# silvadirceu/acoss-1

Hardware: AMD Instinct MI355X
Metric: song-pairs/sec (CSM+Qmax) on 12-d HPCP, ~2000 frames/track; MAP parity (higher is better)
Workload: dtype f32; 1 GPU; covers80-shaped synthetic HPCP (hard corpus), Serra09 CRP+Qmax, all unordered pairs; tracks=164, frames_per_track=2000, m=9, tau=1, oti=True, parallelism=pair-matrix row stripes dp1

## Files before the change

acoss-1_amd/csrc/crp_split.hip:

```cpp
#include <cstdlib>
#include <cstring>
#include <type_traits>

#include "crp_internal.hpp"

__device__ int acoss_writelane(int value, int lane, int old) __asm("llvm.amdgcn.writelane.i32");

namespace acoss {

namespace {

constexpr int kMS = 9;

constexpr unsigned kNone = 0x7fffu;


struct PairView {
  const float* X;
  const float* X2;
  const float* Yr;
  int nq, nr, tau;
  const float* NXq;
  const float* NXr;
  int Mp, Np;
};

__device__ __forceinline__ PairView pair_view(const CrpBatch& B, int p) {
  PairView v;
  const int ta = B.pairs[2 * p], tb = B.pairs[2 * p + 1];
  v.X = B.feats + B.off[ta] * 12;
  v.X2 = B.feats2 ? B.feats2 + (size_t)ta * B.ldn * 24 : nullptr;
  v.Yr = B.yrot + (size_t)p * B.yrot_stride;
  v.nq = B.len[ta];
  v.nr = B.len[tb];
  v.tau = B.tau;
  v.NXq = B.NX + (size_t)ta * B.ldn;
  v.NXr = B.NX + (size_t)tb * B.ldn;
  const int2 dm = B.dims[p];
  v.Mp = dm.x;
  v.Np = dm.y;
  return v;
}

constexpr int kSR = 32;
struct KeyPlanes {
  uint16_t* hr;
  uint16_t* hc;
};

__device__ __forceinline__ float gram12(const f32x4& x0, const f32x4& x1, const f32x4& x2, const f32x4& y0,
                                        const f32x4& y1, const f32x4& y2) {
  float g = 0.0f;
  g = __builtin_fmaf(x0.x, y0.x, g);
  g = __builtin_fmaf(x0.y, y0.y, g);
  g = __builtin_fmaf(x0.z, y0.z, g);
  g = __builtin_fmaf(x0.w, y0.w, g);
  g = __builtin_fmaf(x1.x, y1.x, g);
  g = __builtin_fmaf(x1.y, y1.y, g);
  g = __builtin_fmaf(x1.z, y1.z, g);
  g = __builtin_fmaf(x1.w, y1.w, g);
  g = __builtin_fmaf(x2.x, y2.x, g);
  g = __builtin_fmaf(x2.y, y2.y, g);
  g = __builtin_fmaf(x2.z, y2.z, g);
  g = __builtin_fmaf(x2.w, y2.w, g);
  return g;
}

__device__ __forceinline__ float cell_gram(const PairView& V, int fq, int fr) {
  const f32x4* x = reinterpret_cast<const f32x4*>(V.X + (size_t)fq * 12);
  const f32x4* y = reinterpret_cast<const f32x4*>(V.Yr + (size_t)fr * 12);
  const f32x4 x0 = x[0], x1 = x[1], x2 = x[2], y0 = y[0], y1 = y[1], y2 = y[2];
  return gram12(x0, x1, x2, y0, y1, y2);
}

__device__ __forceinline__ unsigned cell_finish(const PairView& V, int i, int j, float dot) {
  const float d2 = (V.NXq[i] - 2.0f * dot) + V.NXr[j];
  return __builtin_bit_cast(unsigned, d2 > 0.0f ? d2 : 0.0f);
}

__device__ __forceinline__ unsigned cell_key(const PairView& V, int i, int j) {
  float dot = cell_gram(V, i * V.tau, j * V.tau);
#pragma unroll 1
  for (int u = 1; u < kMS; ++u) dot = dot + cell_gram(V, (i + u) * V.tau, (j + u) * V.tau);
  return cell_finish(V, i, j, dot);
}

template <bool ROW>
struct LineCells {
  static constexpr bool kRow = ROW;
  PairView V;
  int fix;
  __device__ __forceinline__ int qi(int e) const { return ROW ? fix : e; }
  __device__ __forceinline__ int rj(int e) const { return ROW ? e : fix; }
  __device__ __forceinline__ unsigned operator()(int e) const { return cell_key(V, qi(e), rj(e)); }
};

typedef float f32x2 __attribute__((ext_vector_type(2)));
typedef __attribute__((address_space(1))) uint16_t gu16;
__device__ __forceinline__ void st_u16(gu16* base, unsigned idx, unsigned v) {
  typedef __attribute__((address_space(1))) char gchar;
  *(gu16*)((gchar*)base + idx * 2u) = (uint16_t)v;
}

__device__ __forceinline__ f32x2 pk_fma(f32x2 a, f32x2 b, f32x2 c) { return __builtin_elementwise_fma(a, b, c); }

constexpr int kSysCols = 56;
constexpr int kThreads = 256;

__device__ __forceinline__ float dpp_shr1(float v) {
  return __builtin_bit_cast(float, __builtin_amdgcn_mov_dpp(__builtin_bit_cast(int, v), 0x138, 0xf, 0xf, true));
}

template <bool PARTIAL>
__device__ __forceinline__ void sweep_body_sys(const PairView& V, int p, int strip, const KeyPlanes& K, int ldr,
                                               int ldc, int64_t kstride, uint16_t* Hr) {
  constexpr int kSteps = kSR + kMS - 1;
  const int i0 = strip * kSR;
  const int rows = PARTIAL ? min(kSR, V.Mp - i0) : kSR;
  const int lane = threadIdx.x & 63;
  const int w = __builtin_amdgcn_readfirstlane(threadIdx.x >> 6);
  uint16_t* Hc = K.hc + (size_t)p * kstride;
  const float* X2b = V.X2 + (size_t)i0 * 24;
  const float* Nq0 = V.NXq + i0;
  auto nqr = [&](int r) {
    const float* base = Nq0;
    asm volatile("" : "+s"(base));
    return *(const __attribute__((address_space(4))) float*)(base + r);
  };
  auto xpair = [&](int kk, f32x2 (&x)[12]) {
    const float* base = X2b;
    asm volatile("" : "+s"(base));
    const cfloat4* q = (const cfloat4*)(base + kk * 24);
#pragma unroll
    for (int c = 0; c < 6; ++c) {
      const f32x4 v = q[c];
      x[2 * c] = f32x2{v.x, v.y};
      x[2 * c + 1] = f32x2{v.z, v.w};
    }
  };
  auto load_y = [&](int jb, f32x4 (&y)[3]) {
    const int f = min(jb + lane, V.nr - 1);
    const f32x4* src = reinterpret_cast<const f32x4*>(V.Yr + (size_t)f * 12);
    y[0] = src[0];
    y[1] = src[1];
    y[2] = src[2];
  };
  const int nblk = (V.Np + kSysCols - 1) / kSysCols;
  f32x4 ynext[3];
  if (w < nblk) load_y(w * kSysCols, ynext);
#pragma unroll 1
  for (int cb = w; cb < nblk; cb += 4) {
    const int jb = cb * kSysCols;
    float y[12];
#pragma unroll
    for (int q = 0; q < 3; ++q) {
      y[4 * q] = ynext[q].x;
      y[4 * q + 1] = ynext[q].y;
      y[4 * q + 2] = ynext[q].z;
      y[4 * q + 3] = ynext[q].w;
    }
    if (cb + 4 < nblk) load_y(jb + 4 * kSysCols, ynext);
    const int col = jb + lane - (kMS - 1);
    const bool valid = lane >= kMS - 1 && col < V.Np;
    const unsigned hcol = valid ? (unsigned)col : (unsigned)(ldr - 1);
    const float ny = valid ? V.NXr[col] : 0.0f;
    gu16* hrow = (gu16*)Hr;
    float A[kMS];
    unsigned kh[16];
    unsigned hw[16];
    f32x2 xb[12];
    xpair(0, xb);
#pragma unroll
    for (int kk = 0; kk < kSteps; kk += 2) {
      f32x2 g2 = pk_fma(xb[0], f32x2{y[0], y[0]}, f32x2{0.0f, 0.0f});
#pragma unroll
      for (int b = 1; b < 12; ++b) g2 = pk_fma(xb[b], f32x2{y[b], y[b]}, g2);
      if (kk + 2 < kSteps) xpair(kk + 2, xb);
      float dots[2];
#pragma unroll
      for (int h = 0; h < 2; ++h) {
        const int k = kk + h;
        const float g = h ? g2.y : g2.x;
#pragma unroll
        for (int u = kMS - 1; u >= 1; --u) {
          const int r = k - u;
          if (r >= 0 && r < kSR) A[u] = dpp_shr1(A[u - 1]) + g;
        }
        if (k < kSR) A[0] = g;
        dots[h] = A[kMS - 1];
      }
      const int r = kk - (kMS - 1);
      if (r >= 0) {
        const f32x2 nq = f32x2{nqr(r), nqr(r + 1)};
        const f32x2 d2 = pk_fma(f32x2{-2.0f, -2.0f}, f32x2{dots[0], dots[1]}, nq) + f32x2{ny, ny};
        unsigned k0 = __builtin_bit_cast(unsigned, d2.x > 0.0f ? d2.x : 0.0f);
        unsigned k1 = __builtin_bit_cast(unsigned, d2.y > 0.0f ? d2.y : 0.0f);
        if (!PARTIAL || r + 1 < rows) {
          st_u16(hrow, hcol, k0 >> 16);
          st_u16(hrow, (unsigned)ldr + hcol, k1 >> 16);
        } else {
          if (r < rows) st_u16(hrow, hcol, k0 >> 16);
          if (r >= rows) k0 = kNone << 16;
          k1 = kNone << 16;
        }
        hrow += 2 * ldr;
        asm volatile("" : "+s"(hrow));
        if (r < 16) {
          kh[r] = k0;
          kh[r + 1] = k1;
        } else {
          hw[r - 16] = __builtin_amdgcn_perm(k0, kh[r - 16], 0x07060302u);
          hw[r - 15] = __builtin_amdgcn_perm(k1, kh[r - 15], 0x07060302u);
        }
      }
    }
    {
      const int m = lane & 3, b = lane & ~3;
      const bool o1 = (m & 1) != 0, o2 = (m & 2) != 0;
      uint32_t T[4][4];
#pragma unroll
      for (int d = 0; d < 4; ++d) {
        const uint32_t x0 = hw[d], x1 = hw[4 + d], x2 = hw[8 + d], x3 = hw[12 + d];
        uint32_t p0 = dpp_u32<0xB1>(x0, x0), p1 = dpp_u32<0xB1>(x1, x1), p2 = dpp_u32<0xB1>(x2, x2),
                 p3 = dpp_u32<0xB1>(x3, x3);
        asm volatile("" : "+v"(p0), "+v"(p1), "+v"(p2), "+v"(p3));
        const uint32_t y0 = o1 ? p1 : x0, y1 = o1 ? x1 : p0, y2 = o1 ? p3 : x2, y3 = o1 ? x3 : p2;
        uint32_t q0 = dpp_u32<0x4E>(y0, y0), q1 = dpp_u32<0x4E>(y1, y1), q2 = dpp_u32<0x4E>(y2, y2),
                 q3 = dpp_u32<0x4E>(y3, y3);
        asm volatile("" : "+v"(q0), "+v"(q1), "+v"(q2), "+v"(q3));
        T[0][d] = o2 ? q2 : y0;
        T[1][d] = o2 ? q3 : y1;
        T[2][d] = o2 ? y2 : q0;
        T[3][d] = o2 ? y3 : q1;
      }
#pragma unroll
      for (int k = 0; k < 4; ++k) {
        const int c = jb + b + k - (kMS - 1);
        if (b + k >= kMS - 1 && c < V.Np)
          reinterpret_cast<uint4*>(Hc + ((size_t)strip * ldc + c) * kSR)[m] = make_uint4(T[k][0], T[k][1], T[k][2], T[k][3]);
      }
    }
  }
  __syncthreads();
  const int padw = (int)((V.Np + 31) & ~31) - V.Np;
  for (int e = threadIdx.x; e < kSR * 32; e += kThreads) {
    const int r = e >> 5, c = e & 31;
    if (c < padw && r < rows) Hr[(size_t)r * ldr + V.Np + c] = (uint16_t)kNone;
  }
}


__device__ __forceinline__ unsigned pk_min_u16(unsigned a, unsigned b) {
  typedef unsigned short u16x2 __attribute__((ext_vector_type(2)));
  return __builtin_bit_cast(unsigned, __builtin_elementwise_min(__builtin_bit_cast(u16x2, a), __builtin_bit_cast(u16x2, b)));
}
__device__ __forceinline__ unsigned pk_max_u16(unsigned a, unsigned b) {
  typedef unsigned short u16x2 __attribute__((ext_vector_type(2)));
  return __builtin_bit_cast(unsigned, __builtin_elementwise_max(__builtin_bit_cast(u16x2, a), __builtin_bit_cast(u16x2, b)));
}
__device__ __forceinline__ unsigned pk_add_u16(unsigned a, unsigned b) {
  typedef unsigned short u16x2 __attribute__((ext_vector_type(2)));
  return __builtin_bit_cast(unsigned, __builtin_bit_cast(u16x2, a) + __builtin_bit_cast(u16x2, b));
}

__device__ __forceinline__ uint32_t gather_flags(uint32_t acc, uint32_t s, int h) {
  return ((s >> (15 - h)) & (0x00010001u << h)) | acc;
}

__device__ __forceinline__ unsigned pk_subsat_u16(unsigned a, unsigned b) {
  typedef unsigned short u16x2 __attribute__((ext_vector_type(2)));
  return __builtin_bit_cast(unsigned, __builtin_elementwise_sub_sat(__builtin_bit_cast(u16x2, a), __builtin_bit_cast(u16x2, b)));
}

template <int NW>
__device__ __forceinline__ unsigned swar_min_greater(const unsigned (&pv)[NW], unsigned x) {
  const unsigned X = ((0x10000u - x - 1u) & 0xffffu) * 0x10001u;
  unsigned a = 0xffffffffu;
#pragma unroll
  for (int h = 0; h < NW; ++h) a = pk_min_u16(a, pk_add_u16(pv[h], X));
  const unsigned d = min(a & 0xffffu, a >> 16);
  return d < kNone - x - 1u ? d + x + 1u : 0xffffffffu;
}

__device__ __forceinline__ uint32_t gather_flags8(uint32_t acc, uint32_t s, int h) {
  return ((s >> (7 - h)) & (0x01010101u << h)) | acc;
}

typedef __attribute__((address_space(3))) unsigned lds_u32;
struct HistAddr {
  unsigned hb, sk;
  __device__ __forceinline__ explicit HistAddr(unsigned* hist) {
    hb = (unsigned)__builtin_amdgcn_readfirstlane((int)(unsigned)(size_t)(lds_u32*)hist);
    sk = hb + 512u + 4u * (threadIdx.x & 63);
  }
};
__device__ __forceinline__ void hist_add(unsigned* hist, const HistAddr& A, unsigned c, bool in) {
  if (in) __hip_atomic_fetch_add(hist + c, 1u, __ATOMIC_RELAXED, __HIP_MEMORY_SCOPE_WAVEFRONT);
}

template <int NW>
__device__ __forceinline__ bool hist_rank_w8(const unsigned (&w8)[NW], unsigned base8, int rho, unsigned* hist,
                                             unsigned* P, int* le, int* less) {
  const int lane = threadIdx.x & 63;
  reinterpret_cast<uint2*>(hist)[lane] = make_uint2(0u, 0u);
  __builtin_amdgcn_wave_barrier();
  const unsigned cmin = base8 == 0u ? 0u : 1u;
  const HistAddr A(hist);
  const unsigned lane1 = (unsigned)(lane + 1) * 0x01010101u;
  const unsigned hbm = A.hb - 4u;
#pragma unroll
  for (int h = 0; h < NW; ++h) {
    const unsigned wp = w8[h] + 0x01010101u;
    const unsigned H = wp & 0x80808080u;
    const unsigned S = wp + ((H - (H >> 7)) & lane1);
#pragma unroll
    for (int k = 0; k < 4; ++k) {
      const unsigned a = hbm + 4u * ((S >> (8 * k)) & 0xffu);
      __hip_atomic_fetch_add((lds_u32*)(size_t)a, 1u, __ATOMIC_RELAXED, __HIP_MEMORY_SCOPE_WAVEFRONT);
    }
  }
  __builtin_amdgcn_wave_barrier();
  const uint2 hv = reinterpret_cast<const uint2*>(hist)[lane];
  const int sl = (int)(hv.x + hv.y);
  const int S = wave_incl_scan(sl);
  const int tot = __builtin_amdgcn_readlane(S, 63);
  const int r = rho;
  if (r < 0 || r >= tot) return false;
  const int E = S - sl;
  const int src = __builtin_ctzll(__ballot(E <= r && r < S));
  const int Es = __builtin_amdgcn_readlane(E, src);
  const int h0 = __builtin_amdgcn_readlane((int)hv.x, src), h1 = __builtin_amdgcn_readlane((int)hv.y, src);
  const bool second = r >= Es + h0;
  if (cmin && src == 0 && !second) return false;
  *P = base8 + 2u * (unsigned)src + (second ? 1u : 0u);
  *less = Es + (second ? h0 : 0);
  *le = *less + (second ? h1 : h0);
  return true;
}

template <int KPL>
struct Line {
  static_assert(KPL == 32, "split word order assumes 32 elements per lane");
  unsigned pv[KPL / 2];
  unsigned w8[KPL / 4];
  unsigned base8;
  bool win;
  __device__ __forceinline__ void build_window(unsigned center) {
    base8 = center > 63u ? center - 63u : 0u;
    win = true;
    const unsigned B2 = base8 * 0x10001u;
    unsigned c[KPL / 2];
#pragma unroll
    for (int h = 0; h < KPL / 2; ++h) c[h] = pk_min_u16(pk_subsat_u16(pv[h], B2), 0x007f007fu);
#pragma unroll
    for (int h = 0; h < KPL / 4; ++h) w8[h] = __builtin_amdgcn_perm(c[h + 8], c[h], 0x06020400u);
  }
  __device__ __forceinline__ bool in_win(unsigned x) const { return win && x >= base8 && x <= base8 + 126u; }
  __device__ __forceinline__ int ebase() const {
    int e = (threadIdx.x & 63) * KPL;
    asm volatile("" : "+v"(e));
    return e;
  }
  __device__ __forceinline__ int elem(int eb, int b) const { return eb + b; }
  static __device__ __forceinline__ int lane_of(int e) { return e / KPL; }
  static __device__ __forceinline__ int bit_of(int e) { return e % KPL; }
  __device__ __forceinline__ unsigned sample() const { return pv[0] & 0xffffu; }
  __device__ __forceinline__ unsigned pfx(int q) const { return q < 16 ? (pv[q] & 0xffffu) : (pv[q - 16] >> 16); }
  template <bool STORED_SPLIT>
  __device__ __forceinline__ void load_lanes(const uint16_t* col0, size_t lane_stride, int n) {
    const int lane = threadIdx.x & 63;
    const int base = lane * KPL;
    const uint16_t* src = col0 + (base < n ? (size_t)lane * lane_stride : (size_t)0);
    win = false;
    base8 = 0u;
    unsigned w[KPL / 2];
#pragma unroll
    for (int q = 0; q < KPL / 8; ++q) {
      const uint4 v = reinterpret_cast<const uint4*>(src)[q];
      w[4 * q + 0] = v.x;
      w[4 * q + 1] = v.y;
      w[4 * q + 2] = v.z;
      w[4 * q + 3] = v.w;
    }
    if (STORED_SPLIT) {
#pragma unroll
      for (int h = 0; h < KPL / 2; ++h) pv[h] = w[h];
    } else {
#pragma unroll
      for (int h = 0; h < KPL / 2; ++h)
        pv[h] = __builtin_amdgcn_perm(w[8 + (h >> 1)], w[h >> 1], (h & 1) ? 0x07060302u : 0x05040100u);
    }
    if (base >= n) {
#pragma unroll
      for (int h = 0; h < KPL / 2; ++h) pv[h] = kNone * 0x10001u;
    }
  }
  __device__ __forceinline__ unsigned cnt8(unsigned x) const {
    const unsigned X4 = (x - base8 + 0x80u) * 0x01010101u;
    unsigned c = 0;
#pragma unroll
    for (int h = 0; h < KPL / 4; ++h) c = __builtin_popcount((X4 - w8[h]) & 0x80808080u) + c;
    return c;
  }
  __device__ __forceinline__ unsigned cnt16(unsigned x) const {
    const unsigned X2 = (x + 0x8000u) * 0x10001u;
    unsigned c = 0;
#pragma unroll
    for (int h = 0; h < KPL / 2; ++h) c = __builtin_popcount((X2 - pv[h]) & 0x80008000u) + c;
    return c;
  }
  __device__ __forceinline__ int count_le(unsigned x) const {
    if (in_win(x)) {
      const unsigned X4 = (x - base8 + 0x80u) * 0x01010101u;
      unsigned c = 0;
#pragma unroll
      for (int h = 0; h < KPL / 4; ++h) c = __builtin_popcount((X4 - w8[h]) & 0x80808080u) + c;
      return wave_sum((int)c);
    }
    const unsigned X2 = (x + 0x8000u) * 0x10001u;
    unsigned c = 0;
#pragma unroll
    for (int h = 0; h < KPL / 2; ++h) c = __builtin_popcount((X2 - pv[h]) & 0x80008000u) + c;
    return wave_sum((int)c);
  }
  __device__ __forceinline__ bool eq_in_win(unsigned P) const {
    return in_win(P) && (P > base8 || base8 == 0u);
  }
  __device__ __forceinline__ uint32_t eq8(unsigned P) const {
    const unsigned PP = (P - base8) * 0x01010101u;
    uint32_t ne8 = 0;
#pragma unroll
    for (int h = 0; h < KPL / 4; ++h) ne8 = gather_flags8(ne8, (w8[h] ^ PP) + 0x7f7f7f7fu, h);
    return ~ne8;
  }
  __device__ __forceinline__ uint32_t eq16(unsigned P) const {
    const unsigned PP = P * 0x10001u;
    uint32_t ne = 0;
#pragma unroll
    for (int h = 0; h < KPL / 2; ++h) ne = gather_flags(ne, (pv[h] ^ PP) + 0x7fff7fffu, h);
    return ~ne;
  }
  __device__ __forceinline__ uint32_t eq_mask(unsigned P) const {
    if (in_win(P) && (P > base8 || base8 == 0u)) {
      const unsigned PP = (P - base8) * 0x01010101u;
      uint32_t ne8 = 0;
#pragma unroll
      for (int h = 0; h < KPL / 4; ++h) ne8 = gather_flags8(ne8, (w8[h] ^ PP) + 0x7f7f7f7fu, h);
      return ~ne8;
    }
    const unsigned PP = P * 0x10001u;
    uint32_t ne = 0;
#pragma unroll
    for (int h = 0; h < KPL / 2; ++h) ne = gather_flags(ne, (pv[h] ^ PP) + 0x7fff7fffu, h);
    return ~ne;
  }
  __device__ __forceinline__ uint32_t le8(unsigned x) const {
    const unsigned X4 = (x - base8 + 0x80u) * 0x01010101u;
    uint32_t le8 = 0;
#pragma unroll
    for (int h = 0; h < KPL / 4; ++h) le8 = gather_flags8(le8, X4 - w8[h], h);
    return le8;
  }
  __device__ __forceinline__ uint32_t le16(unsigned x) const {
    const unsigned X2 = (x + 0x8000u) * 0x10001u;
    uint32_t le = 0;
#pragma unroll
    for (int h = 0; h < KPL / 2; ++h) le = gather_flags(le, X2 - pv[h], h);
    return le;
  }
  __device__ __forceinline__ uint32_t le_mask(unsigned x) const {
    if (in_win(x)) {
      const unsigned X4 = (x - base8 + 0x80u) * 0x01010101u;
      uint32_t le8 = 0;
#pragma unroll
      for (int h = 0; h < KPL / 4; ++h) le8 = gather_flags8(le8, X4 - w8[h], h);
      return le8;
    }
    const unsigned X2 = (x + 0x8000u) * 0x10001u;
    uint32_t le = 0;
#pragma unroll
    for (int h = 0; h < KPL / 2; ++h) le = gather_flags(le, X2 - pv[h], h);
    return le;
  }
  __device__ __forceinline__ void min_max_lane(unsigned* a_io, unsigned* b_io) const {
    unsigned a = *a_io, b = *b_io;
#pragma unroll
    for (int h = 0; h < KPL / 2; ++h) {
      a = pk_min_u16(a, pv[h]);
      b = pk_max_u16(b, pk_add_u16(pv[h], 0x00010001u) & 0x7fff7fffu);
    }
    *a_io = a;
    *b_io = b;
  }
  __device__ __forceinline__ void min_max(unsigned* mn, unsigned* mx) const {
    unsigned a = 0xffffffffu, b = 0u;
    min_max_lane(&a, &b);
    a = min(a & 0xffffu, a >> 16);
    b = max(b & 0xffffu, b >> 16);
    *mn = wave_min_u32(a);
    const unsigned m = wave_max_u32(b);
    *mx = m ? m - 1 : 0u;
  }
  __device__ __forceinline__ unsigned min_greater_lane(unsigned x) const { return swar_min_greater(pv, x); }
  __device__ __forceinline__ unsigned min_greater(unsigned x) const { return wave_min_u32(min_greater_lane(x)); }
  static constexpr int kHalves = 1;
  static constexpr bool kHist = true;
  __device__ __forceinline__ bool hist_rank(unsigned hint, int rho, unsigned* hist, unsigned* P, int* le,
                                            int* less, unsigned* hbase) const {
    if (win) {
      *hbase = base8;
      return hist_rank_w8(w8, base8, rho, hist, P, le, less);
    }
    const int lane = threadIdx.x & 63;
    const unsigned base = hint > 64u ? hint - 64u : 0u;
    *hbase = base;
    reinterpret_cast<uint2*>(hist)[lane] = make_uint2(0u, 0u);
    __builtin_amdgcn_wave_barrier();
    const HistAddr HA(hist);
    unsigned below = 0;
    if (base > 0u) {
      const unsigned X2 = (base - 1u + 0x8000u) * 0x10001u;
#pragma unroll
      for (int h = 0; h < KPL / 2; ++h) below = __builtin_popcount((X2 - pv[h]) & 0x80008000u) + below;
    }
#pragma unroll
    for (int h = 0; h < KPL / 2; ++h) {
#pragma unroll
      for (int half = 0; half < 2; ++half) {
        const unsigned c = (half ? (pv[h] >> 16) : (pv[h] & 0xffffu)) - base;
        hist_add(hist, HA, c, c < 128u);
      }
    }
    const int below_tot = wave_sum((int)below);
    __builtin_amdgcn_wave_barrier();
    const uint2 hv = reinterpret_cast<const uint2*>(hist)[lane];
    const int sl = (int)(hv.x + hv.y);
    const int S = wave_incl_scan(sl);
    const int tot = __builtin_amdgcn_readlane(S, 63);
    const int r = rho - below_tot;
    if (r < 0 || r >= tot) return false;
    const int E = S - sl;
    const int src = __builtin_ctzll(__ballot(E <= r && r < S));
    const int Es = __builtin_amdgcn_readlane(E, src);
// ... 379 lines not shown
    const float d2 = (nq_me - 2.0f * dot) + nr_me;
    G.key = __builtin_bit_cast(unsigned, d2 > 0.0f ? d2 : 0.0f);
  }
  __builtin_amdgcn_wave_barrier();
  return G;
}

template <class LT, class KF>
__device__ __forceinline__ void group_keys2(const LT& L, unsigned P1, int g1, unsigned P2, int g2, const KF& keyf,
                                            WaveLds& W, Group* G1, Group* G2) {
  const int lane = threadIdx.x & 63;
  const int ebase = L.ebase();
  auto m1 = L.eq_mask(P1);
  auto m2 = L.eq_mask(P2);
  const int c1 = popc(m1), c2 = popc(m2);
  const int packed = c1 | (c2 << 16);
  const int sc = wave_incl_scan(packed) - packed;
  int i1 = sc & 0xffff, i2 = g1 + (sc >> 16);
  while (m1) {
    W.list[i1++] = L.elem(ebase, ctz(m1));
    m1 &= m1 - 1;
  }
  while (m2) {
    W.list[i2++] = L.elem(ebase, ctz(m2));
    m2 &= m2 - 1;
  }
  __builtin_amdgcn_wave_barrier();
  const int g = g1 + g2;
  const int e_me = W.list[lane < g ? lane : 0];
  const float nq_me = keyf.V.NXq[keyf.qi(e_me)], nr_me = keyf.V.NXr[keyf.rj(e_me)];
  for (int t = lane; t < kMS * g; t += 64) {
    const int k = t / kMS, u = t - k * kMS;
    const int e = W.list[k];
    W.gv[t] = cell_gram(keyf.V, (keyf.qi(e) + u) * keyf.V.tau, (keyf.rj(e) + u) * keyf.V.tau);
  }
  __builtin_amdgcn_wave_barrier();
  unsigned key = 0xffffffffu;
  if (lane < g) {
    float dot = W.gv[lane * kMS];
#pragma unroll
    for (int u = 1; u < kMS; ++u) dot = dot + W.gv[lane * kMS + u];
    const float d2 = (nq_me - 2.0f * dot) + nr_me;
    key = __builtin_bit_cast(unsigned, d2 > 0.0f ? d2 : 0.0f);
  }
  __builtin_amdgcn_wave_barrier();
  const int elem = lane < g ? e_me : 0;
  *G1 = Group{P1, g1, elem, lane < g1 ? key : 0xffffffffu, 0};
  *G2 = Group{P2, g2, elem, (lane >= g1 && lane < g) ? key : 0xffffffffu, g1};
}

__device__ __forceinline__ unsigned group_min(const Group& G) {
  return wave_min_u32(G.mine(threadIdx.x & 63) ? G.key : 0xffffffffu);
}

__device__ __forceinline__ unsigned group_rank(const Group& G, int rho) {
  const int lane = threadIdx.x & 63;
  int cl = 0, ce = 0;
  for (int k = 0; k < G.g; ++k) {
    const unsigned o = (unsigned)lane_bcast((int)G.key, k);
    cl += o < G.key;
    ce += o == G.key;
  }
  const bool act = lane < G.g;
  const int src = __builtin_ctzll(__ballot(act && cl <= rho && rho < cl + ce));
  return (unsigned)lane_bcast((int)G.key, src);
}

__device__ __forceinline__ void group_rank2(const Group& G, int rho, unsigned* v0, unsigned* v1) {
  const int lane = threadIdx.x & 63;
  int cl = 0, ce = 0;
  for (int k = 0; k < G.g; ++k) {
    const unsigned o = (unsigned)lane_bcast((int)G.key, k);
    cl += o < G.key;
    ce += o == G.key;
  }
  const bool act = lane < G.g;
  const int s0 = __builtin_ctzll(__ballot(act && cl <= rho && rho < cl + ce));
  const int s1 = __builtin_ctzll(__ballot(act && cl <= rho + 1 && rho + 1 < cl + ce));
  *v0 = (unsigned)lane_bcast((int)G.key, s0);
  *v1 = (unsigned)lane_bcast((int)G.key, s1);
}

template <class LT, class F>
__device__ __forceinline__ void group_rounds(const LT& L, unsigned P, int g, WaveLds& W, F fn) {
  const int lane = threadIdx.x & 63;
  auto m = L.eq_mask(P);
  const int cnt = popc(m);
  int idx = wave_incl_scan(cnt) - cnt;
  const int ebase = L.ebase();
  for (int r0 = 0; r0 < g; r0 += 64) {
    while (m && idx < r0 + 64) {
      const int q = ctz(m);
      m &= m - 1;
      W.list[idx - r0] = L.elem(ebase, q);
      ++idx;
    }
    __builtin_amdgcn_wave_barrier();
    if (lane < min(64, g - r0)) fn(W.list[lane]);
    __builtin_amdgcn_wave_barrier();
  }
}

__device__ __forceinline__ unsigned hist_bin_of_rank(const unsigned* hist, int* rho) {
  const int lane = threadIdx.x & 63;
  const unsigned c0 = hist[4 * lane], c1 = hist[4 * lane + 1], c2 = hist[4 * lane + 2], c3 = hist[4 * lane + 3];
  const int tot = (int)(c0 + c1 + c2 + c3);
  const int ex = wave_incl_scan(tot) - tot;
  const int r = *rho;
  int bin = -1, below = ex;
  if (r >= ex && r < ex + tot) {
    if (r < below + (int)c0) {
      bin = 0;
    } else if (r < below + (int)(c0 + c1)) {
      bin = 1;
      below += c0;
    } else if (r < below + (int)(c0 + c1 + c2)) {
      bin = 2;
      below += c0 + c1;
    } else {
      bin = 3;
      below += c0 + c1 + c2;
    }
  }
  const int src = __builtin_ctzll(__ballot(bin >= 0));
  *rho = r - lane_bcast(below, src);
  return (unsigned)(4 * src + lane_bcast(bin, src));
}

template <class LT, class KF>
__device__ __forceinline__ unsigned big_group_rank(const LT& L, unsigned P, int rho, int g, const KF& keyf, WaveLds& W) {
  const int lane = threadIdx.x & 63;
  unsigned* hist = reinterpret_cast<unsigned*>(W.gv);
  unsigned hi8 = 0, lo8 = 0;
#pragma unroll 1
  for (int pass = 0; pass < 2; ++pass) {
    for (int b = lane; b < 256; b += 64) hist[b] = 0u;
    __builtin_amdgcn_wave_barrier();
    group_rounds(L, P, g, W, [&](int e) {
      const unsigned k = keyf(e);
      if (pass == 0)
        atomicAdd(&hist[(k >> 8) & 0xffu], 1u);
      else if (((k >> 8) & 0xffu) == hi8)
        atomicAdd(&hist[k & 0xffu], 1u);
    });
    __builtin_amdgcn_wave_barrier();
    const unsigned bin = hist_bin_of_rank(hist, &rho);
    __builtin_amdgcn_wave_barrier();
    if (pass == 0)
      hi8 = bin;
    else
      lo8 = bin;
  }
  return (P << 16) | (hi8 << 8) | lo8;
}

template <class LT, class KF>
__device__ __forceinline__ unsigned rank_in_prefix(const LT& L, unsigned P, int rho, int g, const KF& keyf, WaveLds& W,
                                   Group* cache) {
  if (g <= 64) {
    if (cache->g < 0 || cache->P != P) *cache = group_keys(L, P, g, keyf, W);
    return group_rank(*cache, rho);
  }
  return big_group_rank(L, P, rho, g, keyf, W);
}

struct Plan {
  unsigned Pl, hbase, Ph2;
  int le, less, gh2, lo, hi;
  float q, lo_f, hi_f;
  bool found, next_ok, both;
};

template <class LT, class KF>
__device__ __forceinline__ Plan line_plan(const LT& L, int n, float kappa, WaveLds& W, Hint* hint) {
  Plan pl;
  pl.q = (float)(n - 1) * kappa;
  pl.lo_f = floorf(pl.q);
  pl.hi_f = ceilf(pl.q);
  pl.lo = (int)pl.lo_f;
  pl.hi = (int)pl.hi_f;
  const int lo = pl.lo, hi = pl.hi;
  unsigned kmin = 0, kmax = 0x7f80u;
  const bool hinted = hint->P != kNoHint;
  if (!hinted) L.min_max(&kmin, &kmax);
  int le = 0, less = 0;
  int passes = 0;
  unsigned Pl = 0u, hbase = 0u;
  bool found = false;
  if constexpr (LT::kHist) {
    if (hinted) found = L.hist_rank(hint->P, lo, W.hist, &Pl, &le, &less, &hbase);
  }
  if (!found) Pl = prefix_of_rank(L, lo, kmin, kmax, n, hint->P, &le, &less, &passes);
  hint->P = Pl;
  hint->dens = hinted ? 0.5f * hint->dens + 0.5f * (float)(le - less) : (float)(le - less);
  pl.Pl = Pl;
  pl.hbase = hbase;
  pl.le = le;
  pl.less = less;
  pl.found = found;
  pl.Ph2 = 0u;
  pl.gh2 = 0;
  pl.next_ok = hi != lo && hi >= le && found && hist_next(W.hist, hbase, Pl, &pl.Ph2, &pl.gh2);
  pl.both = pl.next_ok && le - less <= 64 && (le - less) + pl.gh2 <= 64;
  return pl;
}

template <class LT, class KF>
__device__ __forceinline__ void line_groups(const LT& L, const Plan& pl, const KF& keyf, WaveLds& W, Group* c_lo,
                                            Group* c_hi, unsigned* vlo_o, unsigned* vhi_o) {
  const unsigned Pl = pl.Pl;
  const int le = pl.le, less = pl.less, lo = pl.lo, hi = pl.hi;
  unsigned vlo, vhi;
  if (pl.both) {
    group_keys2(L, Pl, le - less, pl.Ph2, pl.gh2, keyf, W, c_lo, c_hi);
    vlo = group_rank(*c_lo, lo - less);
    vhi = group_min(*c_hi);
  } else if (hi != lo && hi < le && le - less <= 64) {
    *c_lo = group_keys(L, Pl, le - less, keyf, W);
    group_rank2(*c_lo, lo - less, &vlo, &vhi);
  } else {
    vlo = rank_in_prefix(L, Pl, lo - less, le - less, keyf, W, c_lo);
    vhi = vlo;
  }
  if (!pl.both && hi != lo && !(hi < le && le - less <= 64)) {
    if (hi < le) {
      vhi = rank_in_prefix(L, Pl, hi - less, le - less, keyf, W, c_lo);
    } else {
      unsigned Ph;
      int gh;
      if (pl.next_ok) {
        Ph = pl.Ph2;
        gh = pl.gh2;
      } else {
        Ph = L.min_greater(Pl);
        gh = L.count_le(Ph) - le;
      }
      vhi = rank_in_prefix(L, Ph, 0, gh, keyf, W, c_hi);
    }
  }
  *vlo_o = vlo;
  *vhi_o = vhi;
}

__device__ __forceinline__ void plan_threshold(const Plan& pl, unsigned vlo, unsigned vhi, float* thr, float* T) {
  const float slo = sqrt_rn(__builtin_bit_cast(float, vlo));
  float th;
  if (pl.lo_f == pl.hi_f) {
    th = slo;
  } else {
    const float shi = sqrt_rn(__builtin_bit_cast(float, vhi));
    const float aa = slo * (pl.hi_f - pl.q);
    const float bb = shi * (pl.q - pl.lo_f);
    th = aa + bb;
  }
  *thr = th;
  *T = sq_threshold(th);
}

template <class LT, class KF>
__device__ __forceinline__ void line_threshold(const LT& L, int n, float kappa, const KF& keyf, WaveLds& W, Group* c_lo,
                               Group* c_hi, float* thr, float* T, Hint* hint) {
  const Plan pl = line_plan<LT, KF>(L, n, kappa, W, hint);
  unsigned vlo, vhi;
  line_groups(L, pl, keyf, W, c_lo, c_hi, &vlo, &vhi);
  plan_threshold(pl, vlo, vhi, thr, T);
}

template <class LT, class KF>
__device__ __forceinline__ auto le_bits(const LT& L, unsigned Tbits, const KF& keyf, WaveLds& W, const Group& c_lo,
                            const Group& c_hi) {
  const unsigned T16 = Tbits >> 16;
  const int lane = threadIdx.x & 63;
  const auto word = L.le_mask(T16);
  const bool lo_hit = c_lo.g >= 0 && c_lo.P == T16, hi_hit = c_hi.g >= 0 && c_hi.P == T16;
  W.words[lane] = 0xffffffffu;
  if (LT::kHalves == 2) W.words[64 + lane] = 0xffffffffu;
  __builtin_amdgcn_wave_barrier();
  if (lo_hit || hi_hit) {
    const bool cmine = lo_hit ? c_lo.mine(lane) : c_hi.mine(lane);
    const unsigned ckey = lo_hit ? c_lo.key : c_hi.key;
    const int celem = lo_hit ? c_lo.elem : c_hi.elem;
    if (cmine && ckey > Tbits) atomicAnd(&W.words[LT::lane_of(celem)], ~(1u << LT::bit_of(celem)));
  } else {
    const int g = wave_sum(popc(L.eq_mask(T16)));
    if (g == 0) return word;
    if (g <= 64) {
      const Group G = group_keys(L, T16, g, keyf, W);
      if (lane < G.g && G.key > Tbits) atomicAnd(&W.words[LT::lane_of(G.elem)], ~(1u << LT::bit_of(G.elem)));
    } else {
      group_rounds(L, T16, g, W, [&](int e) {
        if (keyf(e) > Tbits) atomicAnd(&W.words[LT::lane_of(e)], ~(1u << LT::bit_of(e)));
      });
    }
  }
  __builtin_amdgcn_wave_barrier();
  if constexpr (LT::kHalves == 2)
    return word & (((uint64_t)W.words[64 + lane] << 32) | W.words[lane]);
  else
    return word & W.words[lane];
}

constexpr int kRowsLds = 4 * (int)sizeof(WaveLds) + kSR * 64 * 4;
constexpr int kRowsLds2 = 4 * (int)sizeof(WaveLds) + kSR * 128 * 4;

template <int J>
__device__ __forceinline__ void transpose_stage(uint32_t (&a)[32]) {
  constexpr uint32_t m = J == 16 ? 0x0000ffffu : J == 8 ? 0x00ff00ffu : J == 4 ? 0x0f0f0f0fu : J == 2 ? 0x33333333u
                                                                                                      : 0x55555555u;
#pragma unroll
  for (int k = 0; k < 32; ++k) {
    if (k & J) continue;
    const uint32_t t = ((a[k] >> J) ^ a[k + J]) & m;
    a[k + J] ^= t;
    a[k] ^= t << J;
  }
}

__device__ __forceinline__ void transpose32(uint32_t (&a)[32]) {
  transpose_stage<16>(a);
  transpose_stage<8>(a);
  transpose_stage<4>(a);
  transpose_stage<2>(a);
  transpose_stage<1>(a);
}

template <int KQ>
struct LineOf {
  using T = LineS<KQ>;
};
template <>
struct LineOf<0> {
  using T = Line<32>;
};
template <>
struct LineOf<2> {
  using T = Line2;
};

template <int NW, int KQ, int RB>
__device__ __forceinline__ void rows_body(const PairView& V, int p, int strip, const uint16_t* Hr, int ldr,
                                          float kappa, float* __restrict__ thr,
                                          float* __restrict__ Tq, int64_t thr_stride, uint32_t* __restrict__ RT,
                                          int64_t rt_stride, int ld, WaveLds* wl, uint32_t (*rowbits)[RB]) {
  using LT = typename LineOf<KQ>::T;
  const int i0 = strip * kSR;
  const int w = __builtin_amdgcn_readfirstlane(threadIdx.x >> 6), lane = threadIdx.x & 63;
  WaveLds& W = wl[w];
  constexpr int RPW = kSR / NW;
  Hint hint{kNoHint, 1.0f};
  auto load_row = [&](LT& Ld, int i) {
    int64_t rowoff = (int64_t)(i - i0) * ldr;
    asm volatile("" : "+s"(rowoff));
    if constexpr (KQ == 0) {
      Ld.template load_lanes<false>(Hr + rowoff, 32, V.Np);
    } else if constexpr (KQ == 2) {
      Ld.A.template load_lanes<false>(Hr + rowoff, 32, V.Np);
      Ld.B.template load_lanes<false>(Hr + rowoff + 2048, 32, V.Np - 2048);
    } else {
      const uint16_t* row = Hr + rowoff;
      Ld.load([&](int e) { return row + (unsigned)e; }, V.Np);
    }
  };
  constexpr bool kPF = KQ != 2;
  auto row = [&](LT& L, int r, auto&& prefetch) {
    const int i = i0 + r;
    uint64_t word = 0;
    if (i < V.Mp) {
      if (hint.P == kNoHint) hint.P = sample_hint(L, V.Np, kappa, W.hist);
      if constexpr (KQ != 8) {
        if (hint.P != kNoHint) L.build_window(hint.P);
      }
      prefetch();
      const LineCells<true> keyf{V, i};
      float th, T;
      Group c_lo, c_hi;
      c_lo.g = c_hi.g = -1;
      line_threshold(L, V.Np, kappa, keyf, W, &c_lo, &c_hi, &th, &T, &hint);
      if (lane == 0) {
        thr[(size_t)p * thr_stride + i] = th;
        Tq[(size_t)p * thr_stride + i] = T;
      }
      word = le_bits(L, __builtin_bit_cast(unsigned, T), keyf, W, c_lo, c_hi);
      if constexpr (KQ == 8 || KQ == 16) word = lane_words<KQ>((uint32_t)word);
    }
    rowbits[r][lane] = (uint32_t)word;
    if constexpr (KQ == 2) rowbits[r][64 + lane] = (uint32_t)(word >> 32);
  };
  const int r1 = (w + 1) * RPW;
  {
    LT Lnext;
    if (kPF && i0 + w * RPW < V.Mp) load_row(Lnext, i0 + w * RPW);
#pragma unroll 1
    for (int r = w * RPW; r < r1; ++r) {
      LT L;
      if (i0 + r < V.Mp) {
        if constexpr (kPF)
          L = Lnext;
        else
          load_row(L, i0 + r);
      }
      row(L, r, [&] {
        if (kPF && r + 1 < r1 && i0 + r + 1 < V.Mp) load_row(Lnext, i0 + r + 1);
      });
    }
  }
  __syncthreads();
  uint32_t* out = RT + (size_t)p * rt_stride + (size_t)strip * ld;
  for (int b = threadIdx.x; 32 * b < V.Np; b += NW * 64) {
    uint32_t a[32];
#pragma unroll
    for (int r = 0; r < 32; ++r) a[r] = rowbits[r][b];
    transpose32(a);
    uint32_t* o = out + 32 * b;
    if (32 * b + 32 <= ld) {
#pragma unroll
      for (int q = 0; q < 32; q += 4) *reinterpret_cast<uint4*>(o + q) = make_uint4(a[q], a[q + 1], a[q + 2], a[q + 3]);
    } else {
#pragma unroll
      for (int q = 0; q < 32; ++q)
        if (32 * b + q < V.Np) o[q] = a[q];
    }
  }
}


constexpr int kSweepWPE = 4;
struct SweepArgs {
  CrpBatch B;
  KeyPlanes K;
  int ldr, ldc;
  int64_t kstride;
  float kappa;
  float* thr;
  float* Tq;
  int64_t thr_stride;
  uint32_t* RT;
  int64_t rt_stride;
  int ld, short_n;
};
struct ColsArgs {
  CrpBatch B;
  KeyPlanes K;
  int ldc;
  int64_t kstride;
  float kappa;
  const uint32_t* RT;
  float* thr;
  float* Tq;
  int64_t thr_stride;
  uint32_t* maskT;
  int64_t mask_stride;
  int ld, short_n;
};
template <int KQ>
constexpr int kSweepLds = KQ == 2 ? kRowsLds2 : kRowsLds;

template <int KQ>
__device__ __forceinline__ void sweep_rows_block(const SweepArgs& A, int strip, int p, char* smem) {
  constexpr int RB = KQ == 2 ? 128 : 64;
  const CrpBatch& B = A.B;
  const KeyPlanes& K = A.K;
  const int ldr = A.ldr, ldc = A.ldc, ld = A.ld, short_n = A.short_n;
  const int64_t kstride = A.kstride, thr_stride = A.thr_stride, rt_stride = A.rt_stride;
  const float kappa = A.kappa;
  float* thr = A.thr;
  float* Tq = A.Tq;
  uint32_t* RT = A.RT;
  const PairView V = pair_view(B, p);
  const int i0 = strip * kSR;
  if (i0 >= V.Mp || V.Np <= 0) return;
  uint16_t* Hr = K.hr + (size_t)p * kstride + (size_t)i0 * ldr;
  if (i0 + kSR <= V.Mp)
    sweep_body_sys<false>(V, p, strip, K, ldr, ldc, kstride, Hr);
  else
    sweep_body_sys<true>(V, p, strip, K, ldr, ldc, kstride, Hr);
  __syncthreads();
  WaveLds* wl = reinterpret_cast<WaveLds*>(smem);
  uint32_t(*rowbits)[RB] = reinterpret_cast<uint32_t(*)[RB]>(smem + 4 * sizeof(WaveLds));
  if (KQ == 8 || V.Np <= short_n)
    rows_body<4, 8, RB>(V, p, strip, Hr, ldr, kappa, thr, Tq, thr_stride, RT, rt_stride, ld, wl, rowbits);
  else if (KQ == 16)
    rows_body<4, 16, RB>(V, p, strip, Hr, ldr, kappa, thr, Tq, thr_stride, RT, rt_stride, ld, wl, rowbits);
  else if (KQ == 2 && V.Np > 2048)
    rows_body<4, 2, RB>(V, p, strip, Hr, ldr, kappa, thr, Tq, thr_stride, RT, rt_stride, ld, wl, rowbits);
  else
    rows_body<4, 0, RB>(V, p, strip, Hr, ldr, kappa, thr, Tq, thr_stride, RT, rt_stride, ld, wl, rowbits);
}

template <int KQ>
__global__ __launch_bounds__(kThreads, kSweepWPE) void k_sweep_rows9(SweepArgs A) {
  __shared__ __attribute__((aligned(16))) char smem[kSweepLds<KQ>];
  sweep_rows_block<KQ>(A, blockIdx.x, blockIdx.y, smem);
}

constexpr int kCPWLong = 2;
constexpr int kCPWShort = 4;
template <int KQ>
constexpr int kCPW = (KQ == 8 || KQ == 16) ? kCPWShort : kCPWLong;
constexpr int kColsWPE = 4;
template <int KQ>
constexpr int kColsPerBlock = 4 * kCPW<KQ>;

template <int KQ>
__device__ __forceinline__ void cols_body(const PairView& V, int p, int j0, int jend, const KeyPlanes& K, int ldc,
                                          int64_t kstride, float kappa, const uint32_t* __restrict__ RT,
                                          float* __restrict__ thr, float* __restrict__ Tq, int64_t thr_stride,
                                          uint32_t* __restrict__ maskT, int64_t mask_stride, int ld, WaveLds& W) {
  constexpr int KPL = 32;
  using LT = typename LineOf<KQ>::T;
  const int lane = threadIdx.x & 63;
  Hint hint{kNoHint, 1.0f};
  auto load_col = [&](LT& Ld, int j) {
    int64_t coloff = (int64_t)p * kstride + (int64_t)j * kSR;
    asm volatile("" : "+s"(coloff));
    if constexpr (KQ == 0) {
      Ld.template load_lanes<true>(K.hc + coloff, (size_t)ldc * kSR, V.Mp);
    } else if constexpr (KQ == 2) {
      Ld.A.template load_lanes<true>(K.hc + coloff, (size_t)ldc * kSR, V.Mp);
      Ld.B.template load_lanes<true>(K.hc + coloff + (size_t)64 * ldc * kSR, (size_t)ldc * kSR, V.Mp - 2048);
    } else {
      const uint16_t* col = K.hc + coloff;
      Ld.load([&](int e) { return col + (unsigned)((e >> 5) * ldc * kSR + (e & 15) * 2 + ((e >> 4) & 1)); }, V.Mp);
    }
  };
  auto column = [&](LT& L, int j) {
    if (hint.P == kNoHint) hint.P = sample_hint(L, V.Mp, kappa, W.hist);
    if constexpr (KQ != 8) {
      if (hint.P != kNoHint) L.build_window(hint.P);
    }
    const size_t w = (size_t)p * mask_stride + (size_t)(lane * KPL < V.Mp ? lane : 0) * ld + j;
    const uint32_t rt = RT[w];
    const size_t w2 = (size_t)p * mask_stride + (size_t)(2048 + lane * KPL < V.Mp ? 64 + lane : 0) * ld + j;
    const uint32_t rt2 = KQ == 2 ? RT[w2] : 0u;
    const LineCells<false> keyf{V, j};
    float th, Tc;
    Group c_lo, c_hi;
    c_lo.g = c_hi.g = -1;
    line_threshold(L, V.Mp, kappa, keyf, W, &c_lo, &c_hi, &th, &Tc, &hint);
    if (lane == 0) {
      thr[(size_t)p * thr_stride + j] = th;
      Tq[(size_t)p * thr_stride + j] = Tc;
    }
    uint64_t bits = le_bits(L, __builtin_bit_cast(unsigned, Tc), keyf, W, c_lo, c_hi);
    if constexpr (KQ == 8 || KQ == 16) bits = lane_words<KQ>((uint32_t)bits);
    if (lane * KPL < V.Mp) maskT[w] = (uint32_t)bits & rt;
    if (KQ == 2 && 2048 + lane * KPL < V.Mp) maskT[w2] = (uint32_t)(bits >> 32) & rt2;
  };
  constexpr bool kPF = KQ != 2;
  {
    LT Lnext;
    if (kPF && j0 < jend) load_col(Lnext, j0);
#pragma unroll 1
    for (int j = j0; j < jend; ++j) {
      LT L;
      if constexpr (kPF)
        L = Lnext;
      else
        load_col(L, j);
      if (kPF && j + 1 < jend) load_col(Lnext, j + 1);
      column(L, j);
    }
  }
}


template <int KQ>
__device__ __forceinline__ void cols_block(const ColsArgs& A, int lin, int ncb, int nblk, WaveLds* wl) {
  const CrpBatch& B = A.B;
  const KeyPlanes& K = A.K;
  const int ldc = A.ldc, ld = A.ld, short_n = A.short_n;
  const int64_t kstride = A.kstride, thr_stride = A.thr_stride, mask_stride = A.mask_stride;
  const float kappa = A.kappa;
  const uint32_t* RT = A.RT;
  float* thr = A.thr;
  float* Tq = A.Tq;
  uint32_t* maskT = A.maskT;
  const int lb = xcd_remap(lin, nblk);
  const int p = lb / ncb;
  const PairView V = pair_view(B, p);
  const int j0 = (lb - p * ncb) * kColsPerBlock<KQ> + __builtin_amdgcn_readfirstlane(threadIdx.x >> 6) * kCPW<KQ>;
  const int jend = min(j0 + kCPW<KQ>, V.Np);
  WaveLds& W = wl[__builtin_amdgcn_readfirstlane(threadIdx.x >> 6)];
  if (KQ == 8 || V.Mp <= short_n)
    cols_body<8>(V, p, j0, jend, K, ldc, kstride, kappa, RT, thr, Tq, thr_stride, maskT, mask_stride, ld, W);
  else if (KQ == 16)
    cols_body<16>(V, p, j0, jend, K, ldc, kstride, kappa, RT, thr, Tq, thr_stride, maskT, mask_stride, ld, W);
  else if (KQ == 2 && V.Mp > 2048)
    cols_body<2>(V, p, j0, jend, K, ldc, kstride, kappa, RT, thr, Tq, thr_stride, maskT, mask_stride, ld, W);
  else
    cols_body<0>(V, p, j0, jend, K, ldc, kstride, kappa, RT, thr, Tq, thr_stride, maskT, mask_stride, ld, W);
}

template <int KQ>
__global__ __launch_bounds__(256, kColsWPE) void k_sel_cols9(ColsArgs A) {
  __shared__ WaveLds wl[4];
  cols_block<KQ>(A, blockIdx.y * gridDim.x + blockIdx.x, gridDim.x, gridDim.x * gridDim.y, wl);
}

}

static int split_kq(int L, int* short_n) {
  static const bool no_short = getenv("ACOSS_NO_SHORT") != nullptr;
  *short_n = no_short ? 0 : 512;
  return L > 2048 ? 2 : (no_short ? 0 : (L <= 512 ? 8 : (L <= 1024 ? 16 : 0)));
}

static SweepArgs sweep_args(const CrpBatch& B, void* kplanes, int ldk, int64_t kstride, int nb,
                            float kappa, float* thr_r, float* T_r, int64_t thr_stride, uint32_t* RT,
                            int64_t mask_stride, int ld, int short_n) {
  const size_t plane = (size_t)nb * kstride;
  const KeyPlanes K{static_cast<uint16_t*>(kplanes), static_cast<uint16_t*>(kplanes) + plane};
  return SweepArgs{B, K, ldk, ldk, kstride, kappa, thr_r, T_r, thr_stride, RT, mask_stride, ld, short_n};
}

static ColsArgs cols_args(const CrpBatch& B, void* kplanes, int ldk, int64_t kstride, int nb, float kappa,
                          const uint32_t* RT, float* thr_c, float* T_c, int64_t thr_stride, uint32_t* maskT,
                          int64_t mask_stride, int ld, int short_n) {
  const size_t plane = (size_t)nb * kstride;
  const KeyPlanes K{static_cast<uint16_t*>(kplanes), static_cast<uint16_t*>(kplanes) + plane};
  return ColsArgs{B, K, ldk, kstride, kappa, RT, thr_c, T_c, thr_stride, maskT, mask_stride, ld, short_n};
}

int launch_crp_split(const CrpBatch& B, int nb, int L, float kappa, void* kplanes, int ldk,
                     int64_t kstride,
                     uint32_t* RT, float* thr_r, float* T_r, float* thr_c, float* T_c, int64_t thr_stride,
                     uint32_t* maskT, int64_t mask_stride, int ld, hipStream_t s) {
  if (B.m != kMS || B.tau != 1 || L > 4096) return 1;
  const int nstrips = (L + kSR - 1) / kSR;
  int short_n;
  const int kq = split_kq(L, &short_n);
  const SweepArgs SA = sweep_args(B, kplanes, ldk, kstride, nb, kappa, thr_r, T_r, thr_stride, RT, mask_stride,
                                  ld, short_n);
  const ColsArgs CA = cols_args(B, kplanes, ldk, kstride, nb, kappa, RT, thr_c, T_c, thr_stride, maskT, mask_stride,
                                ld, short_n);
  auto launch = [&](auto kqc) -> int {
    constexpr int KQ = decltype(kqc)::value;
    prof_begin(PH_SWEEP, s);
    hipLaunchKernelGGL(k_sweep_rows9<KQ>, dim3(nstrips, nb), dim3(kThreads), 0, s, SA);
    ACOSS_LAUNCH_CHECK();
    prof_end(PH_SWEEP, s);
    prof_begin(PH_SEL_COLS, s);
    hipLaunchKernelGGL(k_sel_cols9<KQ>, dim3((L + kColsPerBlock<KQ> - 1) / kColsPerBlock<KQ>, nb), dim3(256), 0, s, CA);
    ACOSS_LAUNCH_CHECK();
    prof_end(PH_SEL_COLS, s);
    return ACOSS_OK;
  };
  if (kq == 8) return launch(std::integral_constant<int, 8>{});
  if (kq == 16) return launch(std::integral_constant<int, 16>{});
  if (kq == 2) return launch(std::integral_constant<int, 2>{});
  return launch(std::integral_constant<int, 0>{});
}

}
```

Before: 88030 song-pairs/s.

## Stage sweep key tiles through LDS for coalesced 16-byte row and column stores

```diff
diff --git a/acoss-1_amd/csrc/crp_split.hip b/acoss-1_amd/csrc/crp_split.hip
--- a/acoss-1_amd/csrc/crp_split.hip
+++ b/acoss-1_amd/csrc/crp_split.hip
@@ -97,15 +97,13 @@
 
 typedef float f32x2 __attribute__((ext_vector_type(2)));
 typedef __attribute__((address_space(1))) uint16_t gu16;
-__device__ __forceinline__ void st_u16(gu16* base, unsigned idx, unsigned v) {
-  typedef __attribute__((address_space(1))) char gchar;
-  *(gu16*)((gchar*)base + idx * 2u) = (uint16_t)v;
-}
 
 __device__ __forceinline__ f32x2 pk_fma(f32x2 a, f32x2 b, f32x2 c) { return __builtin_elementwise_fma(a, b, c); }
 
 constexpr int kSysCols = 56;
 constexpr int kThreads = 256;
+constexpr int kTileBytes = kSR * kSysCols * 2;
+constexpr int kTilePieces = kTileBytes / 16;
 
 __device__ __forceinline__ float dpp_shr1(float v) {
   return __builtin_bit_cast(float, __builtin_amdgcn_mov_dpp(__builtin_bit_cast(int, v), 0x138, 0xf, 0xf, true));
@@ -113,13 +111,14 @@
 
 template <bool PARTIAL>
 __device__ __forceinline__ void sweep_body_sys(const PairView& V, int p, int strip, const KeyPlanes& K, int ldr,
-                                               int ldc, int64_t kstride, uint16_t* Hr) {
+                                               int ldc, int64_t kstride, uint16_t* Hr, char* smem) {
   constexpr int kSteps = kSR + kMS - 1;
   const int i0 = strip * kSR;
   const int rows = PARTIAL ? min(kSR, V.Mp - i0) : kSR;
   const int lane = threadIdx.x & 63;
   const int w = __builtin_amdgcn_readfirstlane(threadIdx.x >> 6);
   uint16_t* Hc = K.hc + (size_t)p * kstride;
+  uint16_t* tile = reinterpret_cast<uint16_t*>(smem + w * kTileBytes);
   const float* X2b = V.X2 + (size_t)i0 * 24;
   const float* Nq0 = V.NXq + i0;
   auto nqr = [&](int r) {
@@ -162,9 +161,7 @@
     if (cb + 4 < nblk) load_y(jb + 4 * kSysCols, ynext);
     const int col = jb + lane - (kMS - 1);
     const bool valid = lane >= kMS - 1 && col < V.Np;
-    const unsigned hcol = valid ? (unsigned)col : (unsigned)(ldr - 1);
     const float ny = valid ? V.NXr[col] : 0.0f;
-    gu16* hrow = (gu16*)Hr;
     float A[kMS];
     unsigned kh[16];
     unsigned hw[16];
@@ -195,16 +192,10 @@
         const f32x2 d2 = pk_fma(f32x2{-2.0f, -2.0f}, f32x2{dots[0], dots[1]}, nq) + f32x2{ny, ny};
         unsigned k0 = __builtin_bit_cast(unsigned, d2.x > 0.0f ? d2.x : 0.0f);
         unsigned k1 = __builtin_bit_cast(unsigned, d2.y > 0.0f ? d2.y : 0.0f);
-        if (!PARTIAL || r + 1 < rows) {
-          st_u16(hrow, hcol, k0 >> 16);
-          st_u16(hrow, (unsigned)ldr + hcol, k1 >> 16);
-        } else {
-          if (r < rows) st_u16(hrow, hcol, k0 >> 16);
+        if (PARTIAL) {
           if (r >= rows) k0 = kNone << 16;
-          k1 = kNone << 16;
+          if (r + 1 >= rows) k1 = kNone << 16;
         }
-        hrow += 2 * ldr;
-        asm volatile("" : "+s"(hrow));
         if (r < 16) {
           kh[r] = k0;
           kh[r + 1] = k1;
@@ -214,31 +205,57 @@
         }
       }
     }
-    {
-      const int m = lane & 3, b = lane & ~3;
-      const bool o1 = (m & 1) != 0, o2 = (m & 2) != 0;
-      uint32_t T[4][4];
-#pragma unroll
-      for (int d = 0; d < 4; ++d) {
-        const uint32_t x0 = hw[d], x1 = hw[4 + d], x2 = hw[8 + d], x3 = hw[12 + d];
-        uint32_t p0 = dpp_u32<0xB1>(x0, x0), p1 = dpp_u32<0xB1>(x1, x1), p2 = dpp_u32<0xB1>(x2, x2),
-                 p3 = dpp_u32<0xB1>(x3, x3);
-        asm volatile("" : "+v"(p0), "+v"(p1), "+v"(p2), "+v"(p3));
-        const uint32_t y0 = o1 ? p1 : x0, y1 = o1 ? x1 : p0, y2 = o1 ? p3 : x2, y3 = o1 ? x3 : p2;
-        uint32_t q0 = dpp_u32<0x4E>(y0, y0), q1 = dpp_u32<0x4E>(y1, y1), q2 = dpp_u32<0x4E>(y2, y2),
-                 q3 = dpp_u32<0x4E>(y3, y3);
-        asm volatile("" : "+v"(q0), "+v"(q1), "+v"(q2), "+v"(q3));
-        T[0][d] = o2 ? q2 : y0;
-        T[1][d] = o2 ? q3 : y1;
-        T[2][d] = o2 ? y2 : q0;
-        T[3][d] = o2 ? y3 : q1;
+    typedef __attribute__((address_space(1))) char gchar;
+    typedef uint32_t u32x4 __attribute__((ext_vector_type(4)));
+    typedef __attribute__((address_space(1))) u32x4 gu4;
+    u32x4* tq = reinterpret_cast<u32x4*>(tile);
+    const int cc = lane - (kMS - 1);
+    if (jb + kSysCols > V.Np) {
+#pragma unroll
+      for (int h = 0; h < 16; ++h) hw[h] = col < V.Np ? hw[h] : kNone * 0x10001u;
+    }
+    if (cc >= 0) {
+      uint16_t* tc = tile + cc;
+#pragma unroll
+      for (int h = 0; h < 16; ++h) {
+        tc[h * kSysCols] = (uint16_t)hw[h];
+        tc[(h + 16) * kSysCols] = (uint16_t)(hw[h] >> 16);
       }
-#pragma unroll
-      for (int k = 0; k < 4; ++k) {
-        const int c = jb + b + k - (kMS - 1);
-        if (b + k >= kMS - 1 && c < V.Np)
-          reinterpret_cast<uint4*>(Hc + ((size_t)strip * ldc + c) * kSR)[m] = make_uint4(T[k][0], T[k][1], T[k][2], T[k][3]);
-      }
+    }
+    __builtin_amdgcn_wave_barrier();
+    u32x4 pr[4], pq[4];
+#pragma unroll
+    for (int k = 0; k < 4; ++k) pr[k] = tq[min(lane + 64 * k, kTilePieces - 1)];
+#pragma unroll
+    for (int k = 0; k < 4; ++k) asm volatile("" : "+v"(pr[k].x), "+v"(pr[k].y), "+v"(pr[k].z), "+v"(pr[k].w));
+#pragma unroll
+    for (int k = 0; k < 4; ++k) {
+      const int t = lane + 64 * k;
+      const int row = t / 7;
+      const int c = jb + 8 * (t - 7 * row);
+      if (t < kTilePieces && c < V.Np && (!PARTIAL || row < rows))
+        *(gu4*)((gchar*)(gu16*)Hr + (unsigned)(row * ldr + c) * 2u) = pr[k];
+    }
+    __builtin_amdgcn_wave_barrier();
+    if (cc >= 0) {
+      const int f = (cc >> 1) & 3;
+#pragma unroll
+      for (int q = 0; q < 4; ++q) tq[cc * 4 + (q ^ f)] = u32x4{hw[4 * q], hw[4 * q + 1], hw[4 * q + 2], hw[4 * q + 3]};
+    }
+    __builtin_amdgcn_wave_barrier();
+#pragma unroll
+    for (int k = 0; k < 4; ++k) {
+      const int t = min(lane + 64 * k, kTilePieces - 1), c = t >> 2;
+      pq[k] = tq[c * 4 + ((t & 3) ^ ((c >> 1) & 3))];
+    }
+#pragma unroll
+    for (int k = 0; k < 4; ++k) asm volatile("" : "+v"(pq[k].x), "+v"(pq[k].y), "+v"(pq[k].z), "+v"(pq[k].w));
+    __builtin_amdgcn_wave_barrier();
+    gu16* hcb = (gu16*)(Hc + ((size_t)strip * ldc + jb) * kSR);
+#pragma unroll
+    for (int k = 0; k < 4; ++k) {
+      const int t = lane + 64 * k;
+      if (t < kTilePieces && jb + (t >> 2) < V.Np) *(gu4*)((gchar*)hcb + (unsigned)t * 16u) = pq[k];
     }
   }
   __syncthreads();
@@ -1224,6 +1241,7 @@
 
 constexpr int kRowsLds = 4 * (int)sizeof(WaveLds) + kSR * 64 * 4;
 constexpr int kRowsLds2 = 4 * (int)sizeof(WaveLds) + kSR * 128 * 4;
+static_assert(4 * kTileBytes <= kRowsLds, "the sweep's staging tiles must fit the row select's LDS");
 
 template <int J>
 __device__ __forceinline__ void transpose_stage(uint32_t (&a)[32]) {
@@ -1346,7 +1364,8 @@
 }
 
 
-constexpr int kSweepWPE = 4;
+template <int KQ>
+constexpr int kSweepWPE = KQ == 8 ? 5 : 4;
 struct SweepArgs {
   CrpBatch B;
   KeyPlanes K;
@@ -1393,9 +1412,9 @@
   if (i0 >= V.Mp || V.Np <= 0) return;
   uint16_t* Hr = K.hr + (size_t)p * kstride + (size_t)i0 * ldr;
   if (i0 + kSR <= V.Mp)
-    sweep_body_sys<false>(V, p, strip, K, ldr, ldc, kstride, Hr);
+    sweep_body_sys<false>(V, p, strip, K, ldr, ldc, kstride, Hr, smem);
   else
-    sweep_body_sys<true>(V, p, strip, K, ldr, ldc, kstride, Hr);
+    sweep_body_sys<true>(V, p, strip, K, ldr, ldc, kstride, Hr, smem);
   __syncthreads();
   WaveLds* wl = reinterpret_cast<WaveLds*>(smem);
   uint32_t(*rowbits)[RB] = reinterpret_cast<uint32_t(*)[RB]>(smem + 4 * sizeof(WaveLds));
@@ -1410,7 +1429,7 @@
 }
 
 template <int KQ>
-__global__ __launch_bounds__(kThreads, kSweepWPE) void k_sweep_rows9(SweepArgs A) {
+__global__ __launch_bounds__(kThreads, kSweepWPE<KQ>) void k_sweep_rows9(SweepArgs A) {
   __shared__ __attribute__((aligned(16))) char smem[kSweepLds<KQ>];
   sweep_rows_block<KQ>(A, blockIdx.x, blockIdx.y, smem);
 }
```

Measured after the change: 90970 song-pairs/s (median of 6 runs). 3.3% higher.
